# reddeupenn/kdtreePathTracerOptimization

Measured on AMD Instinct MI355X. Metric: Mrays/s (800×800, depth 8) + ms/iteration, cornell+dragon; 1/2/4/8 GPU, higher is better.
Workload: dtype f32; 1 GPU; cornell.txt + dragon_5.obj, 800x800, depth 8, bounce cap 8, one 1024-spp frame per step, 8 x 16 iterations in flight, short-stack hybrid KD traversal; scene=cornell, mesh=dragon_5, depth=8, bounce_cap=8, spp_per_frame=1024, kd_nodes=2645, kd_tri_refs=28743, parallelism=single GPU

## Files before the change

### include/kdpt.h

```cpp
#ifndef KDPT_H
#define KDPT_H

#include <stddef.h>
#include <stdint.h>

#ifdef __cplusplus
extern "C" {
#endif

#define KDPT_OK 0
#define KDPT_ERR_ARG -1
#define KDPT_ERR_HIP -2
#define KDPT_ERR_UNSUPPORTED -3
#define KDPT_ERR_IO -4

typedef struct kdpt_geom {
    int type;
    int materialid;
    float translation[3];
    float rotation[3];
    float scale[3];
    float transform[16];
    float inverseTransform[16];
    float invTranspose[16];
// ... 154 lines not shown
#define KDPT_REDUCE_RCCL 0
#define KDPT_REDUCE_COPY 1
int kdpt_comm_unique_id(unsigned char *id);
int kdpt_comm_init(kdpt_ctx *ctx, int nranks, int rank, const unsigned char *id);
int kdpt_comm_library(char *path, int len);
int kdpt_render_frames(kdpt_ctx *ctx, int first_frame, int frames, int spp, int pipeline, int batch, float *out);
int kdpt_render_sharded(const kdpt_scene *scene, const kdpt_options *opt, int ndev, const int *devices,
                        int first_frame, int frames, int spp, int pipeline, int batch, int reduce, float *out);
int kdpt_destroy(kdpt_ctx *ctx);
const char *kdpt_last_error(void);

int kdpt_image_device_ptr(kdpt_ctx *ctx, void **dptr);
int kdpt_debug_paths(kdpt_ctx *ctx, int iter, int stop_depth, kdpt_path_segment *out, int *npaths);
int kdpt_count_iteration(kdpt_ctx *ctx, int iter, unsigned long long *aabb_tri_hit);
int kdpt_count_split(kdpt_ctx *ctx, unsigned long long *aabb_prep_cand);
int kdpt_wave_profile(kdpt_ctx *ctx, unsigned long long *out, int n);
int kdpt_selftest_math(const float *x, int n, float *sin_out, float *cos_out);
int kdpt_selftest_rng(const int *iter_idx_depth, int n, int k, float *u_out);
int kdpt_selftest_rng_draws(int mode, const uint32_t *in, int n, int k, float *out);
int kdpt_selftest_fresnel(const float *cosines, int n, float ior, float *f_out);
int kdpt_selftest_glm(int fn, const float *in, int n, float *out);
int kdpt_selftest_libm(int fn, const float *x, int n, double *out);
int kdpt_selftest_libm_digest(int fn, uint32_t first, unsigned long long count, unsigned long long *digest);

typedef struct kdpt_scene_data kdpt_scene_data;

int kdpt_scene_load(const char *scene_path, const char *obj_path, int res_w, int res_h, int depth,
                    kdpt_scene_data **out);

int kdpt_scene_load_device(const char *scene_path, const char *obj_path, int res_w, int res_h, int depth,
// ... 35 lines not shown
```

### kdtreepathtraceroptimization_amd/csrc/kdpt_device.h

```cpp
#pragma once

#include "kdpt_math.h"

namespace kdpt {

struct DevMaterial {
  float color[3];
  float spec_exponent;
  float spec_color[3];
  float hasReflective;
  float hasRefractive;
  float indexOfRefraction;
  float emittance;
  float transmittance[3];
  float fresnel_R0;
  float pad_[3];
};

struct DevGeom {
  int type;
  int materialid;
  int pad_[2];
  float transform[16];
  float inverseTransform[16];
// ... 59 lines not shown
  int cl_obb;
  int flat_obb;
  float cl_margin, cl_margin_lo, cull_a, cull_b, cull_c;
  const unsigned long long* cl_mask;
  int mask_n;
  const float4* cl_tn;
  const int4* snodes;
  const float4* c_v0;
  const float4* c_e1;
  const float4* c_e2;
  float4 rlo, rhi;
  int trace_mode;
  int early_walk, early_leaf;
  int trip_limit;
  int* fault;
};

struct Ray {
  f3 origin, direction;
  bool isinside;
  float sdepth;
};

KDPT_HD f3 getPointOnRay(const Ray& r, float t) {
  return add(r.origin, scl(normalize(r.direction), t - .0001f));
}

KDPT_HD float boxIntersectionTest(const DevGeom& box, const Ray& r, f3& ip, f3& nrm) {
  Ray q;
  q.origin = mulMV(box.inverseTransform, f4{r.origin.x, r.origin.y, r.origin.z, 1.0f});
// ... 416 lines not shown
  if (nd > beta) return false;
  const float g = -nd - beta;
  return !(g > 0.0f) || tn.w * 1.00001f >= (D - c) * g;
}

KDPT_HD unsigned long long dir_mask_cell(const double* nx, const double* ny, const double* nz, const double* beta,
                                         const double* dthr, const float* krig, const double* D, float Kf) {
  unsigned long long md = 0ull;
  for (int k = 0; k < 64; k++) {
    const double x = nx[k] * D[0] + ny[k] * D[1] + nz[k] * D[2];
    if (x - D[3] <= beta[k] && x + D[3] >= dthr[k] && krig[k] > Kf) md |= 1ull << k;
  }
  return md;
}

#if defined(__HIPCC__) || defined(__HIP__)
constexpr int TRACE_KEYS = 24;
__device__ inline int trace_class(const DevScene& S, f3 o, f3 d) {
  const float4 lo = S.rlo, hi = S.rhi;
  const bool inside = o.x >= lo.x && o.x <= hi.x && o.y >= lo.y && o.y <= hi.y && o.z >= lo.z && o.z <= hi.z;
  const float ix = 1.0f / d.x, iy = 1.0f / d.y, iz = 1.0f / d.z;
  const float t1x = (lo.x - o.x) * ix, t2x = (hi.x - o.x) * ix;
  const float t1y = (lo.y - o.y) * iy, t2y = (hi.y - o.y) * iy;
  const float t1z = (lo.z - o.z) * iz, t2z = (hi.z - o.z) * iz;
  const float tmin = fmaxf(fmaxf(fminf(t1x, t2x), fminf(t1y, t2y)), fminf(t1z, t2z));
  const float tmax = fminf(fminf(fmaxf(t1x, t2x), fmaxf(t1y, t2y)), fmaxf(t1z, t2z));
  const int cls = inside ? 0 : ((tmax >= tmin && tmax >= 0.0f) ? 1 : 2);
  const int oct = (d.x < 0.0f ? 1 : 0) | (d.y < 0.0f ? 2 : 0) | (d.z < 0.0f ? 4 : 0);
  return S.trace_mode == 2 ? oct : (S.trace_mode == 3 ? cls : cls * 8 + oct);
}
// ... 83 lines not shown
    r.hasR = (r.has & 2u) != 0u;
    r.tris = tris;
    r.parent = link16(w3 & 0xffffu);
    r.axis = (int)((w3 >> 16) & 3u);
    r.kc = (w3 >> 21) & 7u;
    return r;
  }
};

enum ProfSlot {
  PROF_NODE_TRIPS, PROF_NODE_CYC, PROF_BIG_SWEEPS, PROF_BIG_CYC, PROF_SMALL_PHASES, PROF_SMALL_ROUNDS,
  PROF_SMALL_CYC, PROF_FINAL_CYC, PROF_SETUP_CYC, PROF_GEOM_CYC, PROF_POST_CYC, PROF_SPARE,
  PROF_BIG_LEAVES, PROF_BIG_CLUSTERS, PROF_BIG_PASS, PROF_BIG_MULTI, PROF_SMALL_PAIRS, PROF_NODE_LEAFWAIT,
  PROF_NODE_DONE, PROF_TAIL_CYC, PROF_TAIL_NODE_DONE, PROF_BIG_SUPERS, PROF_BIG_CULL_CYC, PROF_SLOTS
};

struct ClustersSplit {
  static constexpr bool kSuper = false;
  const float4* lo;
  const float4* hi;
  __device__ float4 lo_of(int c) const { return lo[c]; }
  __device__ float4 hi_of(int c) const { return hi[c]; }
};
struct ClustersInterleaved {
  static constexpr bool kSuper = false;
  const float4* p;
  __device__ float4 lo_of(int c) const { return p[2 * c]; }
  __device__ float4 hi_of(int c) const { return p[2 * c + 1]; }
};
struct ClustersSuper {
// ... 143 lines not shown
  const bool mine = cnt > 0 && rel >= 0 && rel < 64;
  if (mine) slot[rel] = lane + 1;
  wave_lds_sync();
  const int v = wave_incl_scan<true>(slot[lane]);
  if (mine) slot[rel] = 0;
  const int own = v > 0 ? v - 1 : carry;
  carry = __builtin_amdgcn_readlane(own, 63);
  return own;
}

__device__ inline TriData tri_load(const DevScene& S, int i) { return TriData{S.tv0[i], S.te1[i], S.te2[i]}; }


__device__ inline int tri_test(const DevScene& S, int i, f3 o, f3 d, float& bx, float& by, float& bz) {
  return tri_test_v(tri_load(S, i), o, d, bx, by, bz);
}


template <bool HYBRID>
__device__ inline float tri_hit_t_n(float4 n1v, float4 n2v, float4 n3v, f3 o, f3 d, float bx, float by, float bz,
                                    f3& hit, f3& norm) {
  const float w0 = 1 - bx - by;
  norm = normalize(add(add(scl(mk3(n1v.x, n1v.y, n1v.z), w0), scl(mk3(n2v.x, n2v.y, n2v.z), bx)),
                       scl(mk3(n3v.x, n3v.y, n3v.z), by)));
  hit = add(add(o, scl(d, bz)), scl(norm, HYBRID ? 0.0001f : 0.00001f));
  return distance(o, hit);
}

template <bool HYBRID>
__device__ inline float tri_hit_t(const DevScene& S, int i, f3 o, f3 d, float bx, float by, float bz, f3& hit,
// ... 157 lines not shown
  int lstart = 0, lsize = 0, lparent = -1, lclusters = 0;
  uint32_t lkc = 7u;
  float lrestore = 0.0f;
  if (leaf) {
    const NodeRec ln = nodes(cur);
    lstart = ln.triStart;
    lsize = ln.triSize;
    lparent = ln.parent;
    if (NodeSrc::kDerivedBox) {
      lkc = ln.kc;
      lrestore = ln.restore;
    }
    lclusters = (lsize + CLUSTER - 1) / CLUSTER;
    if (S.cl_counts && lsize >= BIG_LEAF) lclusters = S.leaf_cl[lnode].y;
  }
  int r_pass = 0;
  float r_bz = 0.0f;
  int r_lasthit = -1, r_nhit = 0;
  unsigned long long r_best = ~0ull;
  const bool big = leaf && lsize >= BIG_LEAF;
  if (__any(big)) {
    unsigned long long k_pass = 0ull, k_best = ~0ull;
    int k_lasthit = -1, k_nhit = 0;
    auto sweep64 = [&](bool pass, int c, int own) {
      unsigned long long sm = __ballot(pass);
      int s = -1;
      TriData T{};
      if (sm) {
        s = __builtin_ctzll(sm);
        sm &= sm - 1;
        const int ct = __builtin_amdgcn_readlane(c, s) * 64 + lane;
        T = TriData{S.c_v0[ct], S.c_e1[ct], S.c_e2[ct]};
      }
      while (s >= 0) {
        int sn = -1;
        TriData Tn{};
        if (sm) {
          sn = __builtin_ctzll(sm);
          sm &= sm - 1;
          const int ctn = __builtin_amdgcn_readlane(c, sn) * 64 + lane;
          Tn = TriData{S.c_v0[ctn], S.c_e1[ctn], S.c_e2[ctn]};
        }
        if (COUNT) prof_add(WP, PROF_BIG_SWEEPS, 1);
        const int j = __builtin_amdgcn_readlane(own, s);
        const f3 jo = mk3(readlane_f(o.x, j), readlane_f(o.y, j), readlane_f(o.z, j));
        const f3 jd = mk3(readlane_f(d.x, j), readlane_f(d.y, j), readlane_f(d.z, j));
        const int orig = fbits(T.e1.w);
        float bx = 0, by = 0, bzk = 0;
// ... 20 lines not shown
              const float t = tri_hit_t<HYBRID>(S, orig, jo, jd, bx, by, bzk, hp, nn);
              if (t > 0.0f) key = ((unsigned long long)f2u(t) << 32) | (unsigned int)orig;
            }
            const unsigned long long wb = one ? readlane_u64(key, jh) : wave_min_u64(key);
            if (lane == j) {
              k_nhit += __builtin_popcountll(m2);
              k_lasthit = max(k_lasthit, lh);
              k_best = wb < k_best ? wb : k_best;
            }
          }
        }
        s = sn;
        T = Tn;
      }
    };
    auto sweep32 = [&](bool pass, int c, int own) {
      unsigned long long sm = __ballot(pass);
      const bool hi = lane >= 32;
      const unsigned long long hmask = hi ? 0xffffffff00000000ull : 0x00000000ffffffffull;
      auto take = [&]() {
        int t = -1;
        if (sm) {
          t = __builtin_ctzll(sm);
          sm &= sm - 1;
        }
        return t;
      };
      auto load = [&](int a, int b) {
        const int ca = a >= 0 ? __builtin_amdgcn_readlane(c, a) : -1;
        const int cb = b >= 0 ? __builtin_amdgcn_readlane(c, b) : -1;
        const int mc = hi ? cb : ca;
        TriData t{};
        if (mc >= 0) {
          const int ct = mc * 32 + (lane & 31);
          t = TriData{S.c_v0[ct], S.c_e1[ct], S.c_e2[ct]};
        }
        return t;
      };
      int s0 = take(), s1 = take();
      TriData T{};
      if (s0 >= 0) T = load(s0, s1);
      while (s0 >= 0) {
        const int n0 = take(), n1 = take();
        TriData Tn{};
        if (n0 >= 0) Tn = load(n0, n1);
        if (COUNT) prof_add(WP, PROF_BIG_SWEEPS, 1);
        const int j0 = __builtin_amdgcn_readlane(own, s0);
        const int j1 = s1 >= 0 ? __builtin_amdgcn_readlane(own, s1) : j0;
        const f3 o0 = mk3(readlane_f(o.x, j0), readlane_f(o.y, j0), readlane_f(o.z, j0));
        const f3 d0 = mk3(readlane_f(d.x, j0), readlane_f(d.y, j0), readlane_f(d.z, j0));
        const f3 o1 = mk3(readlane_f(o.x, j1), readlane_f(o.y, j1), readlane_f(o.z, j1));
        const f3 d1 = mk3(readlane_f(d.x, j1), readlane_f(d.y, j1), readlane_f(d.z, j1));
        const f3 jo = hi ? o1 : o0, jd = hi ? d1 : d0;
        const int orig = fbits(T.e1.w);
        float bx = 0, by = 0, bzk = 0;
        const int r = tri_test_v(T, jo, jd, bx, by, bzk);
// ... 30 lines not shown
                                 : wave_max_i32(mine && r == 2 ? orig : -1);
              const unsigned long long wb = one ? readlane_u64(key, lh2) : wave_min_u64(mine ? key : ~0ull);
              if (lane == jh) {
                k_nhit += __builtin_popcountll(m2h);
                k_lasthit = max(k_lasthit, lh);
                k_best = wb < k_best ? wb : k_best;
              }
            }
          }
        }
        s0 = n0;
        s1 = n1;
        T = Tn;
      }
    };
    auto sweep = [&](bool pass, int c, int own) {
      if constexpr (CLUSTER == 32) sweep32(pass, c, own);
      else sweep64(pass, c, own);
    };
    const int ncl = big ? lclusters : 0;
    if constexpr (ClusterSrc::kSuper) {
      const int nsp = (ncl + SUPER - 1) / SUPER;
      const int incl = wave_incl_scan<false>(nsp);
      const int P = __builtin_amdgcn_readlane(incl, 63);
      const int excl = incl - nsp;
      W->tbase[lane] = lstart - excl;
      wave_lds_sync();
      if (COUNT) {
        prof_add(WP, PROF_BIG_LEAVES, (unsigned long long)__popcll(__ballot(big)));
        prof_add(WP, PROF_BIG_SUPERS, (unsigned long long)P);
      }
      static_assert(SUPER <= 32 && 64 % SUPER == 0, "super-cluster size");
      unsigned long long* slist = W->best;
      int carry = 0;
// ... 57 lines not shown
            if (S.cl_slab) {
              const CullK ck{S.cl_margin, S.cl_margin_lo, S.cull_a, S.cull_b, S.cull_c};
              const float2 d2 = W->dd[cown];
              const f3 dd = mk3(od.w, d2.x, d2.y);
              if (cp) {
                if (S.cl_obb)
                  cp = cluster_may_pass_obb(rlo, rhi, rn, ru, rv, rw, oo, ii, dd, ck);
                else
                  cp = cluster_may_pass_slab(clusters.lo_of(c), clusters.hi_of(c), clusters.n_of(c), oo, ii, dd, ck);
              }
            } else {
              if (cp) cp = cluster_may_pass(clusters.lo_of(c), clusters.hi_of(c), oo, ii, S.cl_margin);
            }
          }
          if (COUNT) prof_lap(WP, PROF_BIG_CULL_CYC);
          sweep(cp, c, cown);
          if (COUNT) prof_lap(WP, PROF_BIG_CYC);
        }
        wave_lds_sync();
      }
    } else {
      const bool exact = S.cl_mask != nullptr;
      const int cfirst = big ? (NodeSrc::kLeafHoldsCluster ? lstart : S.leaf_cl[lnode].x) : 0;
      const int incl = wave_incl_scan<false>(ncl);
      const int P = __builtin_amdgcn_readlane(incl, 63);
      const int excl = incl - ncl;
      W->tbase[lane] = cfirst - excl;
      wave_lds_sync();
      if (COUNT) {
        prof_add(WP, PROF_BIG_LEAVES, (unsigned long long)__popcll(__ballot(big)));
        prof_add(WP, PROF_BIG_CLUSTERS, (unsigned long long)P);
      }
      int carry = 0;
      for (int B = 0; B < P; B += 64) {
        const int own = pair_owner(W->slot, excl, ncl, B, carry);
        const int c = W->tbase[own] + B + lane;
        bool hit = B + lane < P;
        unsigned long long m = 0ull;
        if (fastAABB) {
          const float4 od = W->od[own];
          const float2 d2 = W->dd[own];
          const f3 oo = mk3(od.x, od.y, od.z), dd = mk3(od.w, d2.x, d2.y);
          const f3 ii = mk3(bpermute_f(invdir.x, own), bpermute_f(invdir.y, own), bpermute_f(invdir.z, own));
          float4 clo = make_float4(0.0f, 0.0f, 0.0f, 0.0f), chi = clo;
          unsigned long long dm = 0ull;
          const bool valid = hit;
          if (valid) {
            if (exact) dm = S.cl_mask[(uint32_t)dir_bucket(dd, S.mask_n) * (uint32_t)S.num_clusters + (uint32_t)c];
            clo = clusters.lo_of(c);
            chi = clusters.hi_of(c);
            hit = cluster_may_pass(clo, chi, oo, ii, S.cl_margin);
          }
          if (S.flat_obb && __any(hit)) {
            if (hit) {
              const float4 cn = S.cl_n[c];
              hit = cluster_may_pass_obb_k(clo, chi, cn, S.cl_u[c], S.cl_v[c], S.cl_w[c], oo, ii, dd,
                                           cn.x * dd.x + cn.y * dd.y + cn.z * dd.z, S.cl_margin);
            }
          }
          if (exact && valid && !hit) m = dm;
        }
        if (COUNT) prof_lap(WP, PROF_BIG_CULL_CYC);
        sweep(hit, c, own);
        if (COUNT) prof_lap(WP, PROF_BIG_CYC);
        if (!exact || !__any(m != 0ull)) continue;
        bool late = false;
        {
          const float4 od = W->od[own];
          const float2 d2 = W->dd[own];
          const f3 oo = mk3(od.x, od.y, od.z), dd = mk3(od.w, d2.x, d2.y);
          const f3 ii = mk3(bpermute_f(invdir.x, own), bpermute_f(invdir.y, own), bpermute_f(invdir.z, own));
          unsigned long long nm = 0ull;
          if (m) {
            const int e0 = c * 64;
            int k0 = __builtin_ctzll(m);
            m &= m - 1;
            float4 t0 = S.cl_tn[e0 + k0];
            const float D = box_miss(clusters.lo_of(c), clusters.hi_of(c), oo, ii);
            while (true) {
              if (danger_needs_test(t0, dd, D, S.cull_c)) nm |= 1ull << k0;
              if (!m) break;
              k0 = __builtin_ctzll(m);
              m &= m - 1;
              t0 = S.cl_tn[e0 + k0];
            }
          }
          if (__any(nm != 0ull)) {
            while (nm && !late) {
              const int e = c * 64 + __builtin_ctzll(nm);
              nm &= nm - 1;
              float bx, by, bz;
              late = tri_test_v(TriData{S.c_v0[e], S.c_e1[e], S.c_e2[e]}, oo, dd, bx, by, bz) >= 1;
            }
          }
        }
        if (COUNT) prof_lap(WP, PROF_BIG_CULL_CYC);
        if (__any(late)) sweep(late, c, own);
        if (COUNT) prof_lap(WP, PROF_BIG_CYC);
      }
    }
    if (big) {
      r_pass = (int)(k_pass >> 32);
      r_bz = u2f((uint32_t)(k_pass & 0xffffffffu));
      r_lasthit = k_lasthit;
      r_nhit = k_nhit;
      r_best = k_best;
    }
  }
  if (COUNT) prof_lap(WP, PROF_BIG_CYC);
  const int sz = (leaf && !big) ? lsize : 0;
  if (__any(sz > 0)) {
    if (COUNT) prof_add(WP, PROF_SMALL_PHASES, 1);
    const int incl = wave_incl_scan<false>(sz);
    const int P = __builtin_amdgcn_readlane(incl, 63);
    const int excl = incl - sz;
    W->tbase[lane] = lstart - excl;
    W->lastPass[lane] = 0ull;
    W->lastHit[lane] = -1;
    W->nhit[lane] = 0;
    W->best[lane] = ~0ull;
    wave_lds_sync();
    if (COUNT) {
      prof_add(WP, PROF_SMALL_ROUNDS, (unsigned long long)((P + 63) / 64));
      prof_add(WP, PROF_SMALL_PAIRS, (unsigned long long)P);
    }
    int carry = 0;
    int owner = pair_owner(W->slot, excl, sz, 0, carry);
    int tri = W->tbase[owner] + lane;
    TriData nxt{};
    if (lane < P) nxt = tri_load(S, tri);
    for (int B = 0; B < P; B += 64) {
      const TriData cur_t = nxt;
      const int cowner = owner, ctri = tri;
      const bool valid = B + lane < P;
      if (B + 64 < P) {
        owner = pair_owner(W->slot, excl, sz, B + 64, carry);
        tri = W->tbase[owner] + B + 64 + lane;
        if (B + 64 + lane < P) nxt = tri_load(S, tri);
      }
      if (valid) {
        const float4 q0 = W->od[cowner];
        const float2 q1 = W->dd[cowner];
        const f3 oo = mk3(q0.x, q0.y, q0.z), dd = mk3(q0.w, q1.x, q1.y);
        float bx, by, bzk;
        const int r = tri_test_v(cur_t, oo, dd, bx, by, bzk);
        if (r >= 1)
          atomicMax(&W->lastPass[cowner], ((unsigned long long)(unsigned int)(ctri + 1) << 32) | f2u(bzk));
        if (r == 2) {
          atomicMax(&W->lastHit[cowner], ctri);
          atomicAdd(&W->nhit[cowner], 1);
          f3 hp, nn;
          const float t = tri_hit_t<HYBRID>(S, ctri, oo, dd, bx, by, bzk, hp, nn);
          if (t > 0.0f) atomicMin(&W->best[cowner], ((unsigned long long)f2u(t) << 32) | (unsigned int)ctri);
        }
      }
    }
    wave_lds_sync();
    if (sz > 0) {
      const unsigned long long lp = W->lastPass[lane];
      r_pass = (int)(lp >> 32);
      r_bz = u2f((uint32_t)(lp & 0xffffffffu));
      r_lasthit = W->lastHit[lane];
      r_nhit = W->nhit[lane];
      r_best = W->best[lane];
    }
    wave_lds_sync();
  }
  if (COUNT) prof_lap(WP, PROF_SMALL_CYC);
  if (leaf) {
    if (COUNT) cnt.tri += lsize;
    if (r_pass > 0) bz = r_bz;
    const int nh = r_nhit;
    if (nh > 0) {
      if (COUNT) cnt.hit += nh;
      h.objMaterialIdx = fbits(S.tv0[r_lasthit].w) + material_size - 1;
      if (HYBRID) {
        for (int rep = 0; rep < (nh > 1 ? 2 : 1); rep++) {
          const bool parVis = (L == 0) ? sink
                              : (L == 1 ? rootv
// ... 208 lines not shown
```

### kdtreepathtraceroptimization_amd/csrc/kdpt_runtime.hip

```cpp
#include <hip/hip_runtime.h>

#include <algorithm>
#include <chrono>
#include <cfloat>
#include <cmath>
#include <cstdio>
#include <cstdlib>
#include <cstring>
#include <memory>
#include <mutex>
#include <string>
#include <vector>

#include <dlfcn.h>
#include <rccl/rccl.h>

#include "../../include/kdpt.h"
#include "kdpt_device.h"
#include "kdpt_clusters.h"

using namespace kdpt;

namespace kdpt_host {
void node_box_matrices(const float* mins, const float* maxs, float* transform16, float* inverse16);
// ... 1474 lines not shown
  int* tile_off = nullptr;
  int* tile_kcounts = nullptr;
  int* tile_koff = nullptr;
  int* perm = nullptr;
  bool trace_order = true;
  bool no_fuse = false;
  bool shade_batch = true;
  bool gen_geoms = true;
  int* ccount0 = nullptr;
  int gen_parity = 0;
  int* cc0_cur = nullptr;
  bool zero_partial = false;
  int chunk_width[3] = {16, 64, 64};
  Counters* counters = nullptr;
  Counters last_profile{};
  unsigned long long* total_segments = nullptr;
  unsigned long long* trace_t = nullptr;
  unsigned long long* trace_total = nullptr;
  double wall_khz = 100000.0;
  int* h_counts = nullptr;
  hipEvent_t ev0 = nullptr, ev1 = nullptr;
  std::vector<hipEvent_t> bounce_ev;
  kdpt_stats stats{};
  bool count_mode = false;
  bool sync_debug = false;
  kdpt_ctx* parent = nullptr;
  std::vector<kdpt_ctx*> slots;
  int slot_batch = 1;
  int next_group = 0;
  bool profile_batches = false;
// ... 865 lines not shown
    c->image_external = true;
  } else if ((rc = dalloc(c, &c->image, 3 * (size_t)c->npix))) {
    return bail(rc);
  }
  if ((rc = dalloc(c, &c->counters, 1)) || (rc = dalloc(c, &c->total_segments, 1)) ||
      (rc = dalloc(c, &c->trace_total, 3)))
    return bail(rc);
  {
    int khz = 0;
    if (hipDeviceGetAttribute(&khz, hipDeviceAttributeWallClockRate, device) == hipSuccess && khz > 0)
      c->wall_khz = khz;
  }
  c->S.trace_mode = 0;
  c->S.early_walk = 16;
  c->S.early_leaf = 1;
  c->trace_order = false;
  if ((rc = setup_trace(c))) return bail(rc);
  c->S.trip_limit = 8 * std::max(c->S.num_nodes, 1) + 64;
  if ((rc = alloc_iteration_events(c))) return bail(rc);
  HIP_TRY(hipDeviceSynchronize());
  if ((rc = kdpt_reset(c))) return bail(rc);
  c->reduce_spin_us = g_reduce_spin_us;
  c->create_ms = std::chrono::duration<double, std::milli>(std::chrono::steady_clock::now() - t_create).count();
  *out = c;
  return KDPT_OK;
}

int kdpt_set_options(kdpt_ctx* c, const kdpt_options* o) {
  if (!c || !o) return fail(KDPT_ERR_ARG, "null arg");
  if (c->parent) return fail(KDPT_ERR_ARG, "not a top-level context");
// ... 43 lines not shown
  if (c->parent) return fail(KDPT_ERR_ARG, "not a top-level context");
  HIP_TRY(hipSetDevice(c->device));
  if (!c->slots.empty()) {
    int rc = kdpt_synchronize(c);
    if (rc) return rc;
    drop_slots(c);
  }
  const std::string k(name);
  const int v = (int)value;
  if (k == "shade_fused") {
    c->no_fuse = v == 0;
  } else if (k == "early_walk") {
    c->S.early_walk = v;
  } else if (k == "early_leaf") {
    c->S.early_leaf = v;
  } else if (k == "shade_batch") {
    c->shade_batch = v != 0;
  } else if (k == "gen_geoms") {
    c->gen_geoms = v != 0;
  } else if (k == "chunk_width0" || k == "chunk_width1" || k == "chunk_width2") {
    c->chunk_width[k.back() - '0'] = std::min(64, std::max(1, v));
  } else if (k == "trace_grid_frac") {
    if (!(value > 0.0 && value <= 1.0)) return fail(KDPT_ERR_ARG, "trace_grid_frac must be in (0, 1]");
    c->trace_grid = std::max(1, (int)(c->full_trace_grid * value));
    c->grid_env = value < 1.0;
  } else if (k == "cluster_obb") {
    c->S.cl_obb = v != 0;
  } else if (k == "flat_obb") {
    c->S.flat_obb = v != 0;
  } else if (k == "super_slab") {
// ... 84 lines not shown

int kdpt_synchronize(kdpt_ctx* c) {
  if (!c) return fail(KDPT_ERR_ARG, "null ctx");
  HIP_TRY(hipSetDevice(c->device));
  HIP_TRY(hipStreamSynchronize(c->stream));
  for (auto sl : c->slots) {
    HIP_TRY(hipStreamSynchronize(sl->stream));
    int rc = check_fault(sl);
    if (rc) return rc;
  }
  if (c->reduce_stream) HIP_TRY(hipStreamSynchronize(c->reduce_stream));
  unregister_host(c);
  int rc = drain_intersect_events(c);
  if (rc) return rc;
  if (c->profile_batches) HIP_TRY(hipMemcpy(&c->last_profile, c->counters, sizeof(Counters), hipMemcpyDeviceToHost));
  return check_fault(c);
}

int kdpt_trace_iteration(kdpt_ctx* c, int frame, int iter) {
  (void)frame;
  if (!c) return fail(KDPT_ERR_ARG, "null ctx");
  HIP_TRY(hipSetDevice(c->device));
  HIP_TRY(hipEventRecord(c->ev0, c->stream));
  int rc = launch_iteration(c, iter, -1, c->count_mode);
  if (rc) return rc;
  HIP_TRY(hipEventRecord(c->ev1, c->stream));
  HIP_TRY(hipMemcpyAsync(c->h_counts, c->counts, sizeof(int) * (c->cap + 3), hipMemcpyDeviceToHost, c->stream));
  HIP_TRY(hipStreamSynchronize(c->stream));
  if (c->h_counts[c->cap + 2]) return fault_error(c, c->h_counts[c->cap + 2]);
  float ms = 0;
// ... 36 lines not shown
      if (rc) return rc;
      c->slots.push_back(sl);
    }
    for (int g = 0; g < depth; g++) {
      hipEvent_t d;
      HIP_TRY(hipEventCreateWithFlags(&d, hipEventDisableTiming));
      c->acc_ev.push_back(d);
    }
  }
  const int ngroups = (int)c->acc_ev.size();
  for (auto sl : c->slots)
    sl->trace_grid =
        c->grid_env ? c->trace_grid : std::max(1, c->trace_grid * 2 / std::min(8, std::max(2, depth)));
  c->stats.intersect_grid_share =
      c->slots.empty() ? 1.0f : (float)c->slots[0]->trace_grid / (float)std::max(1, c->full_trace_grid);
  if (c->profile_batches) HIP_TRY(hipMemsetAsync(c->counters, 0, sizeof(Counters), c->stream));
  bool first = true;
  for (int kb = 0; kb < count; kb += B) {
    const int nb = std::min(B, count - kb);
    const int g = c->next_group % ngroups;
    c->next_group = (g + 1) % ngroups;
    kdpt_ctx* const* grp = &c->slots[(size_t)g * B];
    hipStream_t st = grp[0]->stream;
    int iters[MAXB];
    for (int b = 0; b < nb; b++) {
      iters[b] = first_iter + (kb + b) * stride;
      grp[b]->zero_partial = true;
    }
    std::vector<hipEvent_t>* bev = nullptr;
    if (c->opt.testing_mode) {
      std::vector<hipEvent_t> evs;
// ... 230 lines not shown
  *npaths = n;
  HIP_TRY(hipMemcpy(out, d, sizeof(kdpt_path_segment) * (size_t)n, hipMemcpyDeviceToHost));
  (void)hipFree(d);
  (void)hipFree(scratch);
  return KDPT_OK;
}

int kdpt_count_iteration(kdpt_ctx* c, int iter, unsigned long long* aabb_tri_hit) {
  if (!c || !aabb_tri_hit) return fail(KDPT_ERR_ARG, "null arg");
  HIP_TRY(hipSetDevice(c->device));
  float* saved = c->image;
  float* scratch = nullptr;
  HIP_TRY(hipMalloc((void**)&scratch, sizeof(float) * 3 * (size_t)c->npix));
  HIP_TRY(hipMemsetAsync(scratch, 0, sizeof(float) * 3 * (size_t)c->npix, c->stream));
  HIP_TRY(hipMemsetAsync(c->counters, 0, sizeof(Counters), c->stream));
  c->image = scratch;
  unsigned long long* saved_tot = c->total_segments;
  unsigned long long* scratch_tot = nullptr;
  HIP_TRY(hipMalloc((void**)&scratch_tot, sizeof(unsigned long long)));
  c->total_segments = scratch_tot;
  int rc = launch_iteration(c, iter, -1, true);
  c->total_segments = saved_tot;
  c->image = saved;
  Counters h{};
  if (!rc) {
    HIP_TRY(hipMemcpyAsync(&h, c->counters, sizeof h, hipMemcpyDeviceToHost, c->stream));
    HIP_TRY(hipMemcpyAsync(c->h_counts, c->counts, sizeof(int) * (c->cap + 3), hipMemcpyDeviceToHost, c->stream));
    HIP_TRY(hipStreamSynchronize(c->stream));
    segments_from_counts(c);
    rc = check_fault(c);
  }
  (void)hipFree(scratch);
  (void)hipFree(scratch_tot);
  aabb_tri_hit[0] = h.aabb;
  aabb_tri_hit[1] = h.tri;
  aabb_tri_hit[2] = h.hit;
  c->last_profile = h;
  return rc;
}

int kdpt_count_split(kdpt_ctx* c, unsigned long long* aabb_prep_cand) {
  if (!c || !aabb_prep_cand) return fail(KDPT_ERR_ARG, "null arg");
  aabb_prep_cand[0] = c->last_profile.aabb_prep;
// ... 3 lines not shown

int kdpt_wave_profile(kdpt_ctx* c, unsigned long long* out, int n) {
  if (!c || !out) return fail(KDPT_ERR_ARG, "null arg");
  unsigned long long v[PROF_SLOTS + 5];
  for (int k = 0; k < PROF_SLOTS + 2; k++) v[k] = c->last_profile.wave[k];
  v[PROF_SLOTS + 2] = c->last_profile.aabb;
  v[PROF_SLOTS + 3] = c->last_profile.tri;
  v[PROF_SLOTS + 4] = c->last_profile.hit;
  int k = 0;
  for (; k < n && k < PROF_SLOTS + 5; k++) out[k] = v[k];
  for (int b = 0; b < 64 && k < n; b++, k++) out[k] = c->last_profile.life[b];
  for (int b = 0; b < 64 && k < n; b++, k++) out[k] = c->last_profile.steps[b];
  for (int b = 0; b < 8 && k < n; b++, k++) out[k] = c->last_profile.chord_steps[b];
  for (int b = 0; b < 8 && k < n; b++, k++) out[k] = c->last_profile.chord_n[b];
  return PROF_SLOTS + 5 + 64 + 64 + 16;
}

int kdpt_selftest_math(const float* x, int n, float* so, float* co) {
  float *dx, *ds, *dc;
  HIP_TRY(hipMalloc((void**)&dx, sizeof(float) * n));
  HIP_TRY(hipMalloc((void**)&ds, sizeof(float) * n));
  HIP_TRY(hipMalloc((void**)&dc, sizeof(float) * n));
  HIP_TRY(hipMemcpy(dx, x, sizeof(float) * n, hipMemcpyHostToDevice));
  hipLaunchKernelGGL(k_selftest_math, dim3((n + 255) / 256), dim3(256), 0, 0, dx, n, ds, dc);
  HIP_TRY(hipGetLastError());
  HIP_TRY(hipMemcpy(so, ds, sizeof(float) * n, hipMemcpyDeviceToHost));
  HIP_TRY(hipMemcpy(co, dc, sizeof(float) * n, hipMemcpyDeviceToHost));
  (void)hipFree(dx); (void)hipFree(ds); (void)hipFree(dc);
  return KDPT_OK;
}
// ... 694 lines not shown
```

### kdtreepathtraceroptimization_amd/runtime.py

```python
from __future__ import annotations

import ctypes as C
import os
from dataclasses import dataclass
from typing import Optional

import numpy as np

HERE = os.path.dirname(os.path.abspath(__file__))
LIB_PATH = os.environ.get("KDPT_LIBRARY") or os.path.join(HERE, "libkdpt.so")

KDPT_OK = 0


class KdptError(RuntimeError):
    pass


class Geom(C.Structure):
    _fields_ = [("type", C.c_int), ("materialid", C.c_int), ("translation", C.c_float * 3),
                ("rotation", C.c_float * 3), ("scale", C.c_float * 3), ("transform", C.c_float * 16),
                ("inverseTransform", C.c_float * 16), ("invTranspose", C.c_float * 16)]


# ... 65 lines not shown
                ("shape_materials", C.POINTER(Material)), ("kd_max_depth", C.c_int)]


assert C.sizeof(Geom) == 236 and C.sizeof(Material) == 56 and C.sizeof(Camera) == 84
assert C.sizeof(NodeBare) == 64 and C.sizeof(TriBare) == 76 and C.sizeof(PathSegment) == 56

EXPORTS = [
    "kdpt_default_options", "kdpt_create", "kdpt_trace_iteration", "kdpt_trace_iteration_async", "kdpt_trace_iterations", "kdpt_synchronize",
    "kdpt_read_image", "kdpt_write_pbo", "kdpt_reset", "kdpt_get_stats", "kdpt_destroy", "kdpt_last_error",
    "kdpt_image_device_ptr", "kdpt_debug_paths", "kdpt_count_iteration", "kdpt_count_split", "kdpt_wave_profile", "kdpt_selftest_math", "kdpt_selftest_rng", "kdpt_selftest_rng_draws",
    "kdpt_selftest_fresnel", "kdpt_selftest_libm", "kdpt_selftest_libm_digest", "kdpt_scene_load", "kdpt_scene_build", "kdpt_scene_view", "kdpt_scene_free",
    "kdpt_save_rgb8", "kdpt_save_png", "kdpt_save_hdr", "kdpt_png_encode", "kdpt_write_png", "kdpt_hdr_encode",
    "kdpt_write_hdr", "kdpt_free", "kdpt_set_tuning", "kdpt_selftest_glm", "kdpt_set_options", "kdpt_scene_build_device",
    "kdpt_scene_kd_build_ms", "kdpt_build_kd_device", "kdpt_scene_load_device", "kdpt_trace_config",
    "kdpt_cull_margin", "kdpt_comm_unique_id", "kdpt_comm_init", "kdpt_render_frames", "kdpt_render_sharded",
    "kdpt_comm_library", "kdpt_cull_masks",
]

REDUCE_RCCL, REDUCE_COPY = 0, 1


def set_process_tuning(name: str, value: float):
    lib = load_library()
    _check(lib.kdpt_set_tuning(None, name.encode(), float(value)), f"kdpt_set_tuning(NULL, {name})")

_lib = None


def load_library(path: str = LIB_PATH) -> C.CDLL:
    global _lib
    if _lib is not None:
# ... 13 lines not shown
    lib.kdpt_trace_iteration.argtypes = [C.c_void_p, C.c_int, C.c_int]
    lib.kdpt_trace_iteration_async.argtypes = [C.c_void_p, C.c_int, C.c_int]
    lib.kdpt_trace_iterations.argtypes = [C.c_void_p, C.c_int, C.c_int, C.c_int, C.c_int, C.c_int, C.c_int]
    lib.kdpt_synchronize.argtypes = [C.c_void_p]
    lib.kdpt_read_image.argtypes = [C.c_void_p, P(C.c_float)]
    lib.kdpt_write_pbo.argtypes = [C.c_void_p, C.c_int, P(C.c_uint8)]
    lib.kdpt_reset.argtypes = [C.c_void_p]
    lib.kdpt_get_stats.argtypes = [C.c_void_p, P(Stats)]
    lib.kdpt_destroy.argtypes = [C.c_void_p]
    lib.kdpt_last_error.restype = C.c_char_p
    lib.kdpt_image_device_ptr.argtypes = [C.c_void_p, P(C.c_void_p)]
    lib.kdpt_debug_paths.argtypes = [C.c_void_p, C.c_int, C.c_int, P(PathSegment), P(C.c_int)]
    lib.kdpt_count_iteration.argtypes = [C.c_void_p, C.c_int, P(C.c_ulonglong)]
    if hasattr(lib, "kdpt_count_split"):
        lib.kdpt_count_split.argtypes = [C.c_void_p, P(C.c_ulonglong)]
    lib.kdpt_wave_profile.argtypes = [C.c_void_p, P(C.c_ulonglong), C.c_int]
    lib.kdpt_selftest_math.argtypes = [P(C.c_float), C.c_int, P(C.c_float), P(C.c_float)]
    lib.kdpt_selftest_rng.argtypes = [P(C.c_int), C.c_int, C.c_int, P(C.c_float)]
    lib.kdpt_selftest_fresnel.argtypes = [P(C.c_float), C.c_int, C.c_float, P(C.c_float)]
    lib.kdpt_trace_config.argtypes = [C.c_void_p, P(C.c_int), P(C.c_int), P(C.c_int), P(C.c_longlong)]
    if hasattr(lib, "kdpt_cull_margin"):
        lib.kdpt_cull_margin.argtypes = [C.c_void_p, P(C.c_float), P(C.c_double), P(C.c_int)]
    if hasattr(lib, "kdpt_cull_masks"):
        lib.kdpt_cull_masks.argtypes = [C.c_void_p, P(C.c_int), P(C.c_int), C.c_void_p]
    if hasattr(lib, "kdpt_render_frames"):
        lib.kdpt_comm_unique_id.argtypes = [C.c_void_p]
        lib.kdpt_comm_init.argtypes = [C.c_void_p, C.c_int, C.c_int, C.c_void_p]
        if hasattr(lib, "kdpt_comm_library"):
            lib.kdpt_comm_library.argtypes = [C.c_char_p, C.c_int]
        lib.kdpt_render_frames.argtypes = [C.c_void_p, C.c_int, C.c_int, C.c_int, C.c_int, C.c_int, C.c_void_p]
# ... 333 lines not shown
        _check(self.lib.kdpt_cull_masks(self._ctx, C.byref(n), C.byref(ncl), None), "kdpt_cull_masks")
        if n.value == 0:
            return 0, None
        masks = np.zeros((6 * n.value * n.value, ncl.value), np.uint64)
        _check(self.lib.kdpt_cull_masks(self._ctx, C.byref(n), C.byref(ncl), masks.ctypes.data), "kdpt_cull_masks")
        return n.value, masks

    def trace_grid_share(self) -> float:
        return float(self.stats().intersect_grid_share)

    def count_split(self):
        out = (C.c_ulonglong * 2)()
        _check(self.lib.kdpt_count_split(self._ctx, out), "kdpt_count_split")
        return int(out[0]), int(out[1])

    def wave_profile(self):
        out = (C.c_ulonglong * 256)()
        n = self.lib.kdpt_wave_profile(self._ctx, out, 256)
        _check(0 if n > 0 else n, "kdpt_wave_profile")
        keys = ("node_trips", "node_cycles", "big_sweeps", "big_cycles", "small_phases", "small_rounds",
                "small_cycles", "final_cycles", "setup_cycles", "geom_cycles", "post_cycles", "node_lane_steps",
                "big_leaves", "big_clusters", "big_pass", "big_multi", "small_pairs", "node_leafwait_steps",
                "node_done_steps", "tail_cycles", "tail_node_done_steps", "big_supers", "big_cull_cycles",
                "chunks", "chunk_cycles", "aabb", "tri", "hit")
        prof = dict(zip(keys, (int(out[k]) for k in range(len(keys)))))
        k0 = len(keys)
        if n >= k0 + 64:
            prof["wave_life_10us"] = [int(out[k]) for k in range(k0, k0 + 64)]
        if n >= k0 + 144:
            prof["ray_steps_hist4"] = [int(out[k]) for k in range(k0 + 64, k0 + 128)]
# ... 82 lines not shown
```

Before: 5825 Mrays/s.

## Overlap danger-triangle culling loads with the cluster sweep via async LDS loads

```diff
diff --git a/include/kdpt.h b/include/kdpt.h
--- a/include/kdpt.h
+++ b/include/kdpt.h
@@ -192,6 +192,7 @@
 int kdpt_debug_paths(kdpt_ctx *ctx, int iter, int stop_depth, kdpt_path_segment *out, int *npaths);
 int kdpt_count_iteration(kdpt_ctx *ctx, int iter, unsigned long long *aabb_tri_hit);
 int kdpt_count_split(kdpt_ctx *ctx, unsigned long long *aabb_prep_cand);
+int kdpt_danger_counters(kdpt_ctx *ctx, unsigned long long *out6);
 int kdpt_wave_profile(kdpt_ctx *ctx, unsigned long long *out, int n);
 int kdpt_selftest_math(const float *x, int n, float *sin_out, float *cos_out);
 int kdpt_selftest_rng(const int *iter_idx_depth, int n, int k, float *u_out);
diff --git a/kdtreepathtraceroptimization_amd/csrc/kdpt_device.h b/kdtreepathtraceroptimization_amd/csrc/kdpt_device.h
--- a/kdtreepathtraceroptimization_amd/csrc/kdpt_device.h
+++ b/kdtreepathtraceroptimization_amd/csrc/kdpt_device.h
@@ -97,6 +97,8 @@
   int early_walk, early_leaf;
   int trip_limit;
   int* fault;
+  int danger_overlap, cull_force_late;
+  unsigned long long force_late_m;
 };
 
 struct Ray {
@@ -543,6 +545,25 @@
   return md;
 }
 
+KDPT_HD int nth_set_bit(unsigned long long m, int j) {
+  uint32_t x = (uint32_t)m;
+  int base = 0, c = __builtin_popcount(x);
+  if (j >= c) {
+    j -= c;
+    x = (uint32_t)(m >> 32);
+    base = 32;
+  }
+  for (int w = 16; w >= 1; w >>= 1) {
+    c = __builtin_popcount(x & ((1u << w) - 1u));
+    if (j >= c) {
+      j -= c;
+      x >>= w;
+      base += w;
+    }
+  }
+  return base;
+}
+
 #if defined(__HIPCC__) || defined(__HIP__)
 constexpr int TRACE_KEYS = 24;
 __device__ inline int trace_class(const DevScene& S, f3 o, f3 d) {
@@ -656,6 +677,11 @@
   PROF_BIG_LEAVES, PROF_BIG_CLUSTERS, PROF_BIG_PASS, PROF_BIG_MULTI, PROF_SMALL_PAIRS, PROF_NODE_LEAFWAIT,
   PROF_NODE_DONE, PROF_TAIL_CYC, PROF_TAIL_NODE_DONE, PROF_BIG_SUPERS, PROF_BIG_CULL_CYC, PROF_SLOTS
 };
+enum DangerSlot { DNG_ROUNDS, DNG_ITEMS, DNG_KEPT, DNG_LATE, DNG_PASSES, DNG_PAIRS, DNG_SLOTS };
+static __device__ unsigned long long g_danger_counters[DNG_SLOTS];
+__device__ inline void danger_count(int k, unsigned long long v) {
+  if ((threadIdx.x & 63) == 0 && v) atomicAdd(&g_danger_counters[k], v);
+}
 
 struct ClustersSplit {
   static constexpr bool kSuper = false;
@@ -829,6 +855,90 @@
 
 __device__ inline int tri_test(const DevScene& S, int i, f3 o, f3 d, float& bx, float& by, float& bz) {
   return tri_test_v(tri_load(S, i), o, d, bx, by, bz);
+}
+
+static_assert(offsetof(WaveLeafLDS, lastPass) == 2048 && offsetof(WaveLeafLDS, best) == 2048 + 64 * sizeof(float4),
+              "the danger records' view: lastPass, lastHit and nhit, 1 024 contiguous bytes");
+static_assert(offsetof(WaveLeafLDS, lastPass) % 16 == 0 && sizeof(WaveLeafLDS) % 16 == 0 &&
+                  alignof(WaveLeafLDS) >= 16 && sizeof(float4) == 16,
+              "the danger records' view is 16-byte aligned in every wave's block");
+__device__ inline bool force_late_pair(const DevScene& S, int own, int c) {
+  return S.cull_force_late == 1 || (unsigned long long)(uint32_t)(own + c) * S.force_late_m <= S.force_late_m - 1ull;
+}
+__device__ inline int danger_lane() {
+  int lane = threadIdx.x & 63;
+  asm volatile("" : "+v"(lane));
+  return lane;
+}
+__device__ inline WaveLeafLDS* danger_lds(WaveLeafLDS* W) {
+  auto w3 = (__attribute__((address_space(3))) WaveLeafLDS*)W;
+  asm volatile("" : "+v"(w3));
+  return (WaveLeafLDS*)w3;
+}
+__device__ inline float4* danger_view(WaveLeafLDS* W) { return reinterpret_cast<float4*>(W->lastPass); }
+
+__device__ inline uint32_t danger_find(WaveLeafLDS* W, unsigned long long m, int iexcl, int icnt, int B, int I,
+                                       int& carry) {
+  const int lane = danger_lane();
+  W = danger_lds(W);
+  const int p = pair_owner(W->slot, iexcl, icnt, B, carry);
+  const uint32_t mlo = (uint32_t)__builtin_amdgcn_ds_bpermute(p << 2, (int)(uint32_t)m);
+  const uint32_t mhi = (uint32_t)__builtin_amdgcn_ds_bpermute(p << 2, (int)(uint32_t)(m >> 32));
+  const int pex = __builtin_amdgcn_ds_bpermute(p << 2, iexcl);
+  const int k = B + lane;
+  if (k >= I) return 0u;
+  const int t = nth_set_bit(((unsigned long long)mhi << 32) | mlo, k - pex);
+  return 1u | ((uint32_t)p << 1) | ((uint32_t)t << 7);
+}
+
+__device__ inline void danger_request(const DevScene& S, WaveLeafLDS* W, uint32_t it, int c) {
+  W = danger_lds(W);
+  const int pc = __builtin_amdgcn_ds_bpermute((int)((it >> 1) & 63u) << 2, c);
+  asm volatile("s_waitcnt lgkmcnt(0)" ::: "memory");
+  if (it & 1u) {
+    const float4* src = S.cl_tn + ((size_t)pc * 64 + (it >> 7));
+    __builtin_amdgcn_global_load_lds((const __attribute__((address_space(1))) void*)src,
+                                     (__attribute__((address_space(3))) void*)danger_view(W), 16, 0, 0);
+  }
+}
+
+template <typename ClusterSrc>
+__device__ inline unsigned long long danger_decide(const DevScene& S, const ClusterSrc& clusters, WaveLeafLDS* W,
+                                                   uint32_t it, int c, int own, f3 invdir,
+                                                   unsigned long long& late) {
+  const int lane = danger_lane();
+  W = danger_lds(W);
+  const int p = (int)((it >> 1) & 63u);
+  const int pc = __builtin_amdgcn_ds_bpermute(p << 2, c);
+  const int po = __builtin_amdgcn_ds_bpermute(p << 2, own);
+  const f3 ii = mk3(bpermute_f(invdir.x, po), bpermute_f(invdir.y, po), bpermute_f(invdir.z, po));
+  asm volatile("s_waitcnt vmcnt(0)" ::: "memory");
+  wave_lds_sync();
+  bool keep = false, pass = false;
+  f3 oo = mk3(0.0f, 0.0f, 0.0f), dd = oo;
+  if (it & 1u) {
+    const float4 tn = danger_view(W)[lane];
+    const float4 od = W->od[po];
+    const float2 d2 = W->dd[po];
+    oo = mk3(od.x, od.y, od.z);
+    dd = mk3(od.w, d2.x, d2.y);
+    const float D = box_miss(clusters.lo_of(pc), clusters.hi_of(pc), oo, ii);
+    keep = danger_needs_test(tn, dd, D, S.cull_c);
+  }
+  const unsigned long long km = __ballot(keep);
+  if (km) {
+    if (keep) {
+      const int e = pc * 64 + (int)(it >> 7);
+      float bx, by, bz;
+      pass = tri_test_v(TriData{S.c_v0[e], S.c_e1[e], S.c_e2[e]}, oo, dd, bx, by, bz) >= 1;
+    }
+    unsigned long long pm = __ballot(pass);
+    while (pm) {
+      late |= 1ull << __builtin_amdgcn_readlane(p, __builtin_ctzll(pm));
+      pm &= pm - 1;
+    }
+  }
+  return km;
 }
 
 
@@ -1016,6 +1126,7 @@
     lclusters = (lsize + CLUSTER - 1) / CLUSTER;
     if (S.cl_counts && lsize >= BIG_LEAF) lclusters = S.leaf_cl[lnode].y;
   }
+  constexpr bool kOverlap = !ClusterSrc::kSuper && !NodeSrc::kDerivedBox;
   int r_pass = 0;
   float r_bz = 0.0f;
   int r_lasthit = -1, r_nhit = 0;
@@ -1024,7 +1135,7 @@
   if (__any(big)) {
     unsigned long long k_pass = 0ull, k_best = ~0ull;
     int k_lasthit = -1, k_nhit = 0;
-    auto sweep64 = [&](bool pass, int c, int own) {
+    auto sweep64 = [&](bool pass, int c, int own, auto&& between) {
       unsigned long long sm = __ballot(pass);
       int s = -1;
       TriData T{};
@@ -1034,6 +1145,7 @@
         const int ct = __builtin_amdgcn_readlane(c, s) * 64 + lane;
         T = TriData{S.c_v0[ct], S.c_e1[ct], S.c_e2[ct]};
       }
+      between();
       while (s >= 0) {
         int sn = -1;
         TriData Tn{};
@@ -1084,7 +1196,7 @@
         T = Tn;
       }
     };
-    auto sweep32 = [&](bool pass, int c, int own) {
+    auto sweep32 = [&](bool pass, int c, int own, auto&& between) {
       unsigned long long sm = __ballot(pass);
       const bool hi = lane >= 32;
       const unsigned long long hmask = hi ? 0xffffffff00000000ull : 0x00000000ffffffffull;
@@ -1110,6 +1222,7 @@
       int s0 = take(), s1 = take();
       TriData T{};
       if (s0 >= 0) T = load(s0, s1);
+      between();
       while (s0 >= 0) {
         const int n0 = take(), n1 = take();
         TriData Tn{};
@@ -1170,10 +1283,11 @@
         T = Tn;
       }
     };
-    auto sweep = [&](bool pass, int c, int own) {
-      if constexpr (CLUSTER == 32) sweep32(pass, c, own);
-      else sweep64(pass, c, own);
+    auto sweep = [&](bool pass, int c, int own, auto&& between) {
+      if constexpr (CLUSTER == 32) sweep32(pass, c, own, between);
+      else sweep64(pass, c, own, between);
     };
+    const auto nothing = [] {};
     const int ncl = big ? lclusters : 0;
     if constexpr (ClusterSrc::kSuper) {
       const int nsp = (ncl + SUPER - 1) / SUPER;
@@ -1261,7 +1375,7 @@
             }
           }
           if (COUNT) prof_lap(WP, PROF_BIG_CULL_CYC);
-          sweep(cp, c, cown);
+          sweep(cp, c, cown, nothing);
           if (COUNT) prof_lap(WP, PROF_BIG_CYC);
         }
         wave_lds_sync();
@@ -1272,7 +1386,7 @@
       const int incl = wave_incl_scan<false>(ncl);
       const int P = __builtin_amdgcn_readlane(incl, 63);
       const int excl = incl - ncl;
-      W->tbase[lane] = cfirst - excl;
+      (kOverlap ? danger_lds(W) : W)->tbase[kOverlap ? danger_lane() : lane] = cfirst - excl;
       wave_lds_sync();
       if (COUNT) {
         prof_add(WP, PROF_BIG_LEAVES, (unsigned long long)__popcll(__ballot(big)));
@@ -1292,8 +1406,14 @@
           float4 clo = make_float4(0.0f, 0.0f, 0.0f, 0.0f), chi = clo;
           unsigned long long dm = 0ull;
           const bool valid = hit;
+          int mn = S.mask_n;
+          uint32_t ncm = (uint32_t)S.num_clusters;
+          if (kOverlap) {
+            asm volatile("" : "+v"(mn), "+v"(ncm));
+            mn = __builtin_amdgcn_readfirstlane(mn);
+          }
           if (valid) {
-            if (exact) dm = S.cl_mask[(uint32_t)dir_bucket(dd, S.mask_n) * (uint32_t)S.num_clusters + (uint32_t)c];
+            if (exact) dm = S.cl_mask[(uint32_t)dir_bucket(dd, mn) * ncm + (uint32_t)c];
             clo = clusters.lo_of(c);
             chi = clusters.hi_of(c);
             hit = cluster_may_pass(clo, chi, oo, ii, S.cl_margin);
@@ -1308,10 +1428,68 @@
           if (exact && valid && !hit) m = dm;
         }
         if (COUNT) prof_lap(WP, PROF_BIG_CULL_CYC);
-        sweep(hit, c, own);
+        if (kOverlap && exact && S.danger_overlap) {
+          unsigned long long latem = 0ull;
+          unsigned long long mm = 0ull;
+          uint32_t it = 0u;
+          int I = 0;
+          const auto stage_a = [&] {
+            mm = __ballot(m != 0ull);
+            if (!mm) return;
+            if (COUNT) prof_lap(WP, PROF_BIG_CYC);
+            if (S.cull_force_late > 0)
+              latem = __ballot(m != 0ull && force_late_pair(S, own, c));
+            const int icnt = __popcll(m);
+            const int iincl = wave_incl_scan<false>(icnt);
+            I = __builtin_amdgcn_readlane(iincl, 63);
+            int icarry = 0;
+            it = danger_find(W, m, iincl - icnt, icnt, 0, I, icarry);
+            danger_request(S, W, it, c);
+            if (I > 64) W->best[lane] = m;
+            if (COUNT) prof_lap(WP, PROF_BIG_CULL_CYC);
+          };
+          sweep(hit, c, own, stage_a);
+          if (COUNT) prof_lap(WP, PROF_BIG_CYC);
+          if (!mm) continue;
+          unsigned long long km = danger_decide(S, clusters, W, it, c, own, invdir, latem);
+          if (COUNT) {
+            danger_count(DNG_PASSES, 1);
+            danger_count(DNG_PAIRS, (unsigned long long)__popcll(mm));
+            danger_count(DNG_ITEMS, (unsigned long long)I);
+            danger_count(DNG_ROUNDS, (unsigned long long)((I + 63) / 64));
+            danger_count(DNG_KEPT, (unsigned long long)__popcll(km));
+          }
+          if (I > 64) {
+            const unsigned long long m2 = W->best[lane];
+            const int icnt = __popcll(m2);
+            const int iexcl = wave_incl_scan<false>(icnt) - icnt;
+            int icarry = 0;
+            (void)danger_find(W, m2, iexcl, icnt, 0, I, icarry);
+            for (int Rb = 64; Rb < I; Rb += 64) {
+              const uint32_t itr = danger_find(W, m2, iexcl, icnt, Rb, I, icarry);
+              danger_request(S, W, itr, c);
+              km = danger_decide(S, clusters, W, itr, c, own, invdir, latem);
+              if (COUNT) danger_count(DNG_KEPT, (unsigned long long)__popcll(km));
+            }
+          }
+          if (COUNT) prof_lap(WP, PROF_BIG_CULL_CYC);
+          if (latem) {
+            if (COUNT) danger_count(DNG_LATE, (unsigned long long)__popcll(latem));
+            sweep(((latem >> lane) & 1ull) != 0ull, c, own, nothing);
+          }
+          if (COUNT) prof_lap(WP, PROF_BIG_CYC);
+          continue;
+        }
+        sweep(hit, c, own, nothing);
         if (COUNT) prof_lap(WP, PROF_BIG_CYC);
         if (!exact || !__any(m != 0ull)) continue;
-        bool late = false;
+        bool late = S.cull_force_late > 0 && m != 0ull && force_late_pair(S, own, c);
+        if (COUNT) {
+          danger_count(DNG_PASSES, 1);
+          danger_count(DNG_PAIRS, (unsigned long long)__popcll(__ballot(m != 0ull)));
+          danger_count(DNG_ITEMS,
+                   (unsigned long long)__builtin_amdgcn_readlane(wave_incl_scan<false>(__popcll(m)), 63));
+        }
         {
           const float4 od = W->od[own];
           const float2 d2 = W->dd[own];
@@ -1332,6 +1510,9 @@
               t0 = S.cl_tn[e0 + k0];
             }
           }
+          if (COUNT)
+            danger_count(DNG_KEPT,
+                     (unsigned long long)__builtin_amdgcn_readlane(wave_incl_scan<false>(__popcll(nm)), 63));
           if (__any(nm != 0ull)) {
             while (nm && !late) {
               const int e = c * 64 + __builtin_ctzll(nm);
@@ -1342,7 +1523,8 @@
           }
         }
         if (COUNT) prof_lap(WP, PROF_BIG_CULL_CYC);
-        if (__any(late)) sweep(late, c, own);
+        if (COUNT) danger_count(DNG_LATE, (unsigned long long)__popcll(__ballot(late)));
+        if (__any(late)) sweep(late, c, own, nothing);
         if (COUNT) prof_lap(WP, PROF_BIG_CYC);
       }
     }
@@ -1358,58 +1540,62 @@
   const int sz = (leaf && !big) ? lsize : 0;
   if (__any(sz > 0)) {
     if (COUNT) prof_add(WP, PROF_SMALL_PHASES, 1);
+    WaveLeafLDS* const Ws = kOverlap ? danger_lds(W) : W;
+    const int ls = kOverlap ? danger_lane() : lane;
+    int neg1 = -1;
+    if (kOverlap) asm volatile("" : "+v"(neg1));
     const int incl = wave_incl_scan<false>(sz);
     const int P = __builtin_amdgcn_readlane(incl, 63);
     const int excl = incl - sz;
-    W->tbase[lane] = lstart - excl;
-    W->lastPass[lane] = 0ull;
-    W->lastHit[lane] = -1;
-    W->nhit[lane] = 0;
-    W->best[lane] = ~0ull;
+    Ws->tbase[ls] = lstart - excl;
+    Ws->lastPass[ls] = 0ull;
+    Ws->lastHit[ls] = neg1;
+    Ws->nhit[ls] = 0;
+    Ws->best[ls] = ((unsigned long long)(uint32_t)neg1 << 32) | (uint32_t)neg1;
     wave_lds_sync();
     if (COUNT) {
       prof_add(WP, PROF_SMALL_ROUNDS, (unsigned long long)((P + 63) / 64));
       prof_add(WP, PROF_SMALL_PAIRS, (unsigned long long)P);
     }
     int carry = 0;
-    int owner = pair_owner(W->slot, excl, sz, 0, carry);
-    int tri = W->tbase[owner] + lane;
+    int owner = pair_owner(Ws->slot, excl, sz, 0, carry);
+    int tri = Ws->tbase[owner] + ls;
     TriData nxt{};
-    if (lane < P) nxt = tri_load(S, tri);
+    if (ls < P) nxt = tri_load(S, tri);
     for (int B = 0; B < P; B += 64) {
       const TriData cur_t = nxt;
       const int cowner = owner, ctri = tri;
-      const bool valid = B + lane < P;
+      const bool valid = B + ls < P;
       if (B + 64 < P) {
-        owner = pair_owner(W->slot, excl, sz, B + 64, carry);
-        tri = W->tbase[owner] + B + 64 + lane;
-        if (B + 64 + lane < P) nxt = tri_load(S, tri);
+        owner = pair_owner(Ws->slot, excl, sz, B + 64, carry);
+        tri = Ws->tbase[owner] + B + 64 + ls;
+        if (B + 64 + ls < P) nxt = tri_load(S, tri);
       }
       if (valid) {
-        const float4 q0 = W->od[cowner];
-        const float2 q1 = W->dd[cowner];
+        const float4 q0 = Ws->od[cowner];
+        const float2 q1 = Ws->dd[cowner];
         const f3 oo = mk3(q0.x, q0.y, q0.z), dd = mk3(q0.w, q1.x, q1.y);
         float bx, by, bzk;
         const int r = tri_test_v(cur_t, oo, dd, bx, by, bzk);
         if (r >= 1)
-          atomicMax(&W->lastPass[cowner], ((unsigned long long)(unsigned int)(ctri + 1) << 32) | f2u(bzk));
+          atomicMax(&Ws->lastPass[cowner], ((unsigned long long)(unsigned int)(ctri + 1) << 32) | f2u(bzk));
         if (r == 2) {
-          atomicMax(&W->lastHit[cowner], ctri);
-          atomicAdd(&W->nhit[cowner], 1);
+          atomicMax(&Ws->lastHit[cowner], ctri);
+          atomicAdd(&Ws->nhit[cowner], 1);
           f3 hp, nn;
           const float t = tri_hit_t<HYBRID>(S, ctri, oo, dd, bx, by, bzk, hp, nn);
-          if (t > 0.0f) atomicMin(&W->best[cowner], ((unsigned long long)f2u(t) << 32) | (unsigned int)ctri);
+          if (t > 0.0f) atomicMin(&Ws->best[cowner], ((unsigned long long)f2u(t) << 32) | (unsigned int)ctri);
         }
       }
     }
     wave_lds_sync();
     if (sz > 0) {
-      const unsigned long long lp = W->lastPass[lane];
+      const unsigned long long lp = Ws->lastPass[ls];
       r_pass = (int)(lp >> 32);
       r_bz = u2f((uint32_t)(lp & 0xffffffffu));
-      r_lasthit = W->lastHit[lane];
-      r_nhit = W->nhit[lane];
-      r_best = W->best[lane];
+      r_lasthit = Ws->lastHit[ls];
+      r_nhit = Ws->nhit[ls];
+      r_best = Ws->best[ls];
     }
     wave_lds_sync();
   }
diff --git a/kdtreepathtraceroptimization_amd/csrc/kdpt_runtime.hip b/kdtreepathtraceroptimization_amd/csrc/kdpt_runtime.hip
--- a/kdtreepathtraceroptimization_amd/csrc/kdpt_runtime.hip
+++ b/kdtreepathtraceroptimization_amd/csrc/kdpt_runtime.hip
@@ -1512,6 +1512,7 @@
   int chunk_width[3] = {16, 64, 64};
   Counters* counters = nullptr;
   Counters last_profile{};
+  unsigned long long last_danger[DNG_SLOTS] = {};
   unsigned long long* total_segments = nullptr;
   unsigned long long* trace_t = nullptr;
   unsigned long long* trace_total = nullptr;
@@ -2407,6 +2408,9 @@
   c->S.trace_mode = 0;
   c->S.early_walk = 16;
   c->S.early_leaf = 1;
+  c->S.danger_overlap = 1;
+  c->S.cull_force_late = 0;
+  c->S.force_late_m = 0ull;
   c->trace_order = false;
   if ((rc = setup_trace(c))) return bail(rc);
   c->S.trip_limit = 8 * std::max(c->S.num_nodes, 1) + 64;
@@ -2480,6 +2484,12 @@
     c->S.early_walk = v;
   } else if (k == "early_leaf") {
     c->S.early_leaf = v;
+  } else if (k == "danger_overlap") {
+    c->S.danger_overlap = v != 0;
+  } else if (k == "cull_force_late") {
+    if (v < 0) return fail(KDPT_ERR_ARG, "cull_force_late must be >= 0 (0: off)");
+    c->S.cull_force_late = v;
+    c->S.force_late_m = v > 1 ? ~0ull / (unsigned long long)v + 1ull : 0ull;
   } else if (k == "shade_batch") {
     c->shade_batch = v != 0;
   } else if (k == "gen_geoms") {
@@ -2594,6 +2604,8 @@
   int rc = drain_intersect_events(c);
   if (rc) return rc;
   if (c->profile_batches) HIP_TRY(hipMemcpy(&c->last_profile, c->counters, sizeof(Counters), hipMemcpyDeviceToHost));
+  if (c->profile_batches)
+    HIP_TRY(hipMemcpyFromSymbol(c->last_danger, HIP_SYMBOL(g_danger_counters), sizeof c->last_danger));
   return check_fault(c);
 }
 
@@ -2660,7 +2672,11 @@
         c->grid_env ? c->trace_grid : std::max(1, c->trace_grid * 2 / std::min(8, std::max(2, depth)));
   c->stats.intersect_grid_share =
       c->slots.empty() ? 1.0f : (float)c->slots[0]->trace_grid / (float)std::max(1, c->full_trace_grid);
-  if (c->profile_batches) HIP_TRY(hipMemsetAsync(c->counters, 0, sizeof(Counters), c->stream));
+  if (c->profile_batches) {
+    HIP_TRY(hipMemsetAsync(c->counters, 0, sizeof(Counters), c->stream));
+    const unsigned long long zero[DNG_SLOTS] = {};
+    HIP_TRY(hipMemcpyToSymbol(HIP_SYMBOL(g_danger_counters), zero, sizeof zero));
+  }
   bool first = true;
   for (int kb = 0; kb < count; kb += B) {
     const int nb = std::min(B, count - kb);
@@ -2921,6 +2937,10 @@
   HIP_TRY(hipMalloc((void**)&scratch, sizeof(float) * 3 * (size_t)c->npix));
   HIP_TRY(hipMemsetAsync(scratch, 0, sizeof(float) * 3 * (size_t)c->npix, c->stream));
   HIP_TRY(hipMemsetAsync(c->counters, 0, sizeof(Counters), c->stream));
+  {
+    const unsigned long long zero[DNG_SLOTS] = {};
+    HIP_TRY(hipMemcpyToSymbol(HIP_SYMBOL(g_danger_counters), zero, sizeof zero));
+  }
   c->image = scratch;
   unsigned long long* saved_tot = c->total_segments;
   unsigned long long* scratch_tot = nullptr;
@@ -2934,6 +2954,7 @@
     HIP_TRY(hipMemcpyAsync(&h, c->counters, sizeof h, hipMemcpyDeviceToHost, c->stream));
     HIP_TRY(hipMemcpyAsync(c->h_counts, c->counts, sizeof(int) * (c->cap + 3), hipMemcpyDeviceToHost, c->stream));
     HIP_TRY(hipStreamSynchronize(c->stream));
+    HIP_TRY(hipMemcpyFromSymbol(c->last_danger, HIP_SYMBOL(g_danger_counters), sizeof c->last_danger));
     segments_from_counts(c);
     rc = check_fault(c);
   }
@@ -2967,6 +2988,12 @@
   for (int b = 0; b < 8 && k < n; b++, k++) out[k] = c->last_profile.chord_steps[b];
   for (int b = 0; b < 8 && k < n; b++, k++) out[k] = c->last_profile.chord_n[b];
   return PROF_SLOTS + 5 + 64 + 64 + 16;
+}
+
+int kdpt_danger_counters(kdpt_ctx* c, unsigned long long* out6) {
+  if (!c || !out6) return fail(KDPT_ERR_ARG, "null arg");
+  for (int k = 0; k < DNG_SLOTS; k++) out6[k] = c->last_danger[k];
+  return KDPT_OK;
 }
 
 int kdpt_selftest_math(const float* x, int n, float* so, float* co) {
diff --git a/kdtreepathtraceroptimization_amd/runtime.py b/kdtreepathtraceroptimization_amd/runtime.py
--- a/kdtreepathtraceroptimization_amd/runtime.py
+++ b/kdtreepathtraceroptimization_amd/runtime.py
@@ -103,7 +103,7 @@
     "kdpt_write_hdr", "kdpt_free", "kdpt_set_tuning", "kdpt_selftest_glm", "kdpt_set_options", "kdpt_scene_build_device",
     "kdpt_scene_kd_build_ms", "kdpt_build_kd_device", "kdpt_scene_load_device", "kdpt_trace_config",
     "kdpt_cull_margin", "kdpt_comm_unique_id", "kdpt_comm_init", "kdpt_render_frames", "kdpt_render_sharded",
-    "kdpt_comm_library", "kdpt_cull_masks",
+    "kdpt_comm_library", "kdpt_cull_masks", "kdpt_danger_counters",
 ]
 
 REDUCE_RCCL, REDUCE_COPY = 0, 1
@@ -147,6 +147,8 @@
     lib.kdpt_count_iteration.argtypes = [C.c_void_p, C.c_int, P(C.c_ulonglong)]
     if hasattr(lib, "kdpt_count_split"):
         lib.kdpt_count_split.argtypes = [C.c_void_p, P(C.c_ulonglong)]
+    if hasattr(lib, "kdpt_danger_counters"):
+        lib.kdpt_danger_counters.argtypes = [C.c_void_p, P(C.c_ulonglong)]
     lib.kdpt_wave_profile.argtypes = [C.c_void_p, P(C.c_ulonglong), C.c_int]
     lib.kdpt_selftest_math.argtypes = [P(C.c_float), C.c_int, P(C.c_float), P(C.c_float)]
     lib.kdpt_selftest_rng.argtypes = [P(C.c_int), C.c_int, C.c_int, P(C.c_float)]
@@ -510,6 +512,12 @@
         _check(self.lib.kdpt_count_split(self._ctx, out), "kdpt_count_split")
         return int(out[0]), int(out[1])
 
+    def danger_counters(self) -> dict:
+        out = (C.c_ulonglong * 6)()
+        _check(self.lib.kdpt_danger_counters(self._ctx, out), "kdpt_danger_counters")
+        keys = ("rounds", "items", "kept", "late", "passes", "pairs")
+        return dict(zip(keys, (int(v) for v in out)))
+
     def wave_profile(self):
         out = (C.c_ulonglong * 256)()
         n = self.lib.kdpt_wave_profile(self._ctx, out, 256)
```

Result: no change. 5882 Mrays/s (median of 6 runs) (+1.0%).
